# EntityOfCode/eoc-tfhe

Hardware: AMD Instinct MI355X
Metric: gate bootstraps/sec (HomNAND) (higher is better)
Workload: dtype f64

## Files before the change

eoc_tfhe_amd/csrc/kernels.hip.h:

```cpp
#pragma once
#include <hip/hip_runtime.h>
#include <stdint.h>
#include <type_traits>

namespace eoc {

typedef double d2 __attribute__((ext_vector_type(2)));

constexpr int kN = 1024;
constexpr int kNH = 512;
constexpr int kScr = 568;
constexpr int kTwF1 = 0;
constexpr int kTwF2 = 32;
constexpr int kTwI1 = 32 + 256;
constexpr int kTwI0 = 32 + 256 + 32;
constexpr int kTwEntries = 32 + 256 + 32 + 256;

#define EOC_FMA(a, b, c) __builtin_fma((a), (b), (c))

#define EOC_SQRT_HALF 0x1.6a09e667f3bcdp-1
#define EOC_E128_RE 0x1.d906bcf328d46p-1
#define EOC_E128_IM 0x1.87de2a6aea963p-2
#define EOC_E64_RE 0x1.f6297cff75cb0p-1
#define EOC_E64_IM 0x1.8f8b83c69a60bp-3
// ... 759 lines not shown
        EOC_SGB(EOC_M_DSW, 1);
        EOC_SGB(EOC_M_VALU, 5);
    }
    EOC_SGB(EOC_M_VALU, 16);
    EOC_SGB(EOC_M_DSR, 8);
    EOC_SB();
#pragma unroll
    for (int r = 0; r < 8; r++) scr[f12(lane * 8 + r)] = xb[r];
    wave_lds_fence();
    t21_read(xb, scr, lane);
    tw_load(t0, tw + kTwI0 + lane, 64);
    wave_lds_fence();
    inv_pass10(xa, t1);
#pragma unroll
    for (int k = 0; k < 8; k++) {
        EOC_SGB(EOC_M_DSW, 1);
        EOC_SGB(EOC_M_VALU, 4);
    }
    EOC_SGB(EOC_M_DSR, 12);
    EOC_SGB(EOC_M_VALU, 40);
    EOC_SB();
#pragma unroll
    for (int r = 0; r < 8; r++) scr[72 * hi + 8 * r + lo] = xa[r];
    wave_lds_fence();
    t10_read(xa, scr, lane);
    inv_pass10(xb, t1);
#pragma unroll
    for (int k = 0; k < 8; k++) {
        EOC_SGB(EOC_M_DSW, 1);
        EOC_SGB(EOC_M_VALU, 4);
    }
    EOC_SGB(EOC_M_DSR, 8);
    EOC_SGB(EOC_M_VALU, 40);
    EOC_SB();
#pragma unroll
    for (int r = 0; r < 8; r++) scr[72 * hi + 8 * r + lo] = xb[r];
    wave_lds_fence();
    t10_read(xb, scr, lane);
#pragma unroll
    for (int r = 0; r < 8; r++) ut[r] = s_twist[lane + 64 * r];
    wave_lds_fence();
    inv_pass10(xa, t0);
#pragma unroll
    for (int k = 0; k < 8; k++) {
        EOC_SGB(EOC_M_DSW, 1);
        EOC_SGB(EOC_M_VALU, 4);
    }
    EOC_SGB(EOC_M_DSR, 16);
    EOC_SGB(EOC_M_VALU, 40);
    EOC_SB();
    inv_pass10(xb, t0);
}

constexpr int kBRWideJobsPerWG = 2;
constexpr int kBRWideLds = (kTwEntries + kNH + kBRWideJobsPerWG * kScr) * 16 + kBRWideJobsPerWG * kAbarLds;


template <int BGBIT = 0, bool SABAR = false>
__global__ __launch_bounds__(64 * kBRWideJobsPerWG, 2) void k_blind_rotate_wide(BRArgs A, const d2 *__restrict__ g_tw,
                                                              const d2 *__restrict__ g_twist)
{
    constexpr bool TV = false, MANY = false, ENC = false;
    const int32_t *const tv = nullptr;
    const uint32_t tv_rows = 1, n_tables = 1;
#include "blind_rotate_wide.inc"
}
template <int BGBIT = 0, bool SABAR = false>
__global__ __launch_bounds__(64 * kBRWideJobsPerWG, 2) void k_blind_rotate_wide_tv(BRArgs A, const d2 *__restrict__ g_tw,
                                                                 const d2 *__restrict__ g_twist,
                                                                 const int32_t *__restrict__ tv, uint32_t tv_rows)
{
    constexpr bool TV = true, MANY = false, ENC = false;
    const uint32_t n_tables = 1;
#include "blind_rotate_wide.inc"
}
template <int BGBIT = 0, bool SABAR = false>
__global__ __launch_bounds__(64 * kBRWideJobsPerWG, 2) void k_lut_many_wide(BRArgs A, const d2 *__restrict__ g_tw,
                                                                            const d2 *__restrict__ g_twist,
                                                                            const int32_t *__restrict__ tv, uint32_t tv_rows,
                                                                            uint32_t n_tables)
{
    constexpr bool TV = true, MANY = true, ENC = false;
#include "blind_rotate_wide.inc"
}
template <int BGBIT = 0, bool SABAR = false>
__global__ __launch_bounds__(64 * kBRWideJobsPerWG, 2) void k_br_enc_wide(BRArgs A, const d2 *__restrict__ g_tw,
                                                                          const d2 *__restrict__ g_twist,
                                                                          const int32_t *__restrict__ tv, uint32_t tv_rows)
{
    constexpr bool TV = true, MANY = false, ENC = true;
    const uint32_t n_tables = 1;
#include "blind_rotate_wide.inc"
}

constexpr int KS_GT = 64;

struct KSArgs {
    const int32_t *ksk;
    const int32_t *u;
    uint32_t *ubar;
    int n, n1p, t, basebit;
    uint32_t S;
    GateDesc desc0;
    int inline_desc;
    int32_t mu;
};

__global__ __launch_bounds__(256) void k_ks_init(const GateDesc *__restrict__ descs, KSArgs A)
{
    const GateDesc d = A.inline_desc ? A.desc0 : descs[blockIdx.y];
    const uint32_t s = blockIdx.x;
    const uint32_t job = d.job_base + s;
    const int32_t *u1 = A.u + (size_t)job * (kN + 1);
    const bool mux = d.op == OP_MUX;
    const int32_t *u2 = u1 + (size_t)A.S * (kN + 1);
    const uint32_t prec_offset = 1u << (32 - (1 + A.basebit * A.t));
    for (int j = threadIdx.x; j < kN; j += 256) {
        uint32_t v = (uint32_t)u1[j];
        if (mux) v += (uint32_t)u2[j];
        A.ubar[(size_t)job * kN + j] = v + prec_offset;
    }
    int32_t *o = d.out + (size_t)s * (A.n + 1);
    for (int m = threadIdx.x; m < A.n; m += 256) o[m] = 0;
    if (threadIdx.x == 0) {
        uint32_t b = (uint32_t)u1[kN];
        if (mux) b += (uint32_t)u2[kN] + (uint32_t)A.mu;
        o[A.n] = (int32_t)b;
    }
}

typedef int i4 __attribute__((ext_vector_type(4)));

template <int T, int NWV, int IW>
struct KS3Cfg {
    static constexpr int NT = 64 * NWV;
    static constexpr int ROWI = 64 + 4;
    static constexpr int TABI = 16 * ROWI;
    static constexpr int WAVE_I = 2 * TABI;
    static constexpr int RED_I = 64 * ROWI;
    static constexpr int TAB_BYTES = NWV * WAVE_I * 4, RED_BYTES = (NWV > 1 ? NWV / 2 : 1) * RED_I * 4;
    static constexpr int LDS_BYTES = TAB_BYTES > RED_BYTES ? TAB_BYTES : RED_BYTES;
    static constexpr int NPAIR = T / 2;
    static constexpr int NSTAGE = IW * NPAIR;
    static constexpr int SLICE_I = NWV * IW;
    static constexpr int NS = kN / SLICE_I;
};

template <int T, int NWV, int IW>
__global__ __launch_bounds__(64 * NWV, 4) void k_keyswitch_waves(const GateDesc *__restrict__ descs, KSArgs A)
{
    typedef KS3Cfg<T, NWV, IW> C;
    static_assert(T % 2 == 0 && kN % C::SLICE_I == 0 && (NWV & (NWV - 1)) == 0, "shape");
    static_assert((NWV * C::WAVE_I - C::TABI) * 4 < 65536, "ds_write_addtid_b32 takes its base from M0[15:0]");
    extern __shared__ __attribute__((aligned(16))) unsigned char smem[];
    int *s_all = reinterpret_cast<int *>(smem);
    if ((uint32_t)(uintptr_t)smem != 0u) __builtin_trap();

    const GateDesc d = A.inline_desc ? A.desc0 : descs[blockIdx.y];
    const uint32_t ntiles = (A.S + 63) / 64, ncb = (uint32_t)A.n1p / 64u;
    const uint32_t tile = blockIdx.x % ntiles, rest = blockIdx.x / ntiles;
    const uint32_t cb = rest % ncb, slice = rest / ncb;
    const uint32_t s0 = tile * 64;
    const int tid = threadIdx.x, lane = tid & 63;
    const int w = __builtin_amdgcn_readfirstlane(tid >> 6);
    const bool valid = s0 + lane < A.S;
    const uint32_t job = d.job_base + (valid ? s0 + lane : A.S - 1);
    const int i0 = (int)slice * C::SLICE_I + w * IW;

    int *s_tab = s_all + w * C::WAVE_I;
    const size_t n1p = (size_t)A.n1p;
    int kr[6];
    for (int k = lane; k < 2 * C::ROWI; k += 64) s_tab[(k / C::ROWI) * C::TABI + k % C::ROWI] = 0;
    const uint32_t tab_lds = (uint32_t)(uintptr_t)s_tab;
    auto stage_load = [&](int st) {
        const int i = i0 + st / C::NPAIR, j0 = 2 * (st % C::NPAIR);
        const int *src = A.ksk + ((size_t)i * T + j0) * 3 * n1p + cb * 64 + lane;
#pragma unroll
        for (int k = 0; k < 6; k++) kr[k] = src[k * n1p];
    };
#define EOC_KS_ROW(BUF, D1, D2) ((BUF) * C::TABI * 4 + ((D1) * 4 + (D2)) * C::ROWI * 4)
    auto stage_store = [&](int buf) {
        const int a1 = kr[0], a2 = kr[1], a3 = kr[2], b1 = kr[3], b2 = kr[4], b3 = kr[5];
        const uint32_t base = tab_lds + (uint32_t)buf * (C::TABI * 4);
        uint32_t m0_saved;
        asm volatile("s_mov_b32 %0, m0\n\t"
                     "s_mov_b32 m0, %1\n\t"
                     "s_nop 1\n\t"
                     "ds_write_addtid_b32 %2 offset:%17\n\t"
                     "ds_write_addtid_b32 %3 offset:%18\n\t"
                     "ds_write_addtid_b32 %4 offset:%19\n\t"
                     "ds_write_addtid_b32 %5 offset:%20\n\t"
                     "ds_write_addtid_b32 %6 offset:%21\n\t"
                     "ds_write_addtid_b32 %7 offset:%22\n\t"
                     "ds_write_addtid_b32 %8 offset:%23\n\t"
                     "ds_write_addtid_b32 %9 offset:%24\n\t"
                     "ds_write_addtid_b32 %10 offset:%25\n\t"
                     "ds_write_addtid_b32 %11 offset:%26\n\t"
                     "ds_write_addtid_b32 %12 offset:%27\n\t"
                     "ds_write_addtid_b32 %13 offset:%28\n\t"
                     "ds_write_addtid_b32 %14 offset:%29\n\t"
                     "ds_write_addtid_b32 %15 offset:%30\n\t"
                     "ds_write_addtid_b32 %16 offset:%31\n\t"
                     "s_mov_b32 m0, %0"
                     : "=&s"(m0_saved)
                     : "s"(base), "v"(b1), "v"(b2), "v"(b3), "v"(a1), "v"(a1 + b1), "v"(a1 + b2), "v"(a1 + b3), "v"(a2),
                       "v"(a2 + b1), "v"(a2 + b2), "v"(a2 + b3), "v"(a3), "v"(a3 + b1), "v"(a3 + b2), "v"(a3 + b3),
                       "n"(EOC_KS_ROW(0, 0, 1)), "n"(EOC_KS_ROW(0, 0, 2)), "n"(EOC_KS_ROW(0, 0, 3)), "n"(EOC_KS_ROW(0, 1, 0)),
                       "n"(EOC_KS_ROW(0, 1, 1)), "n"(EOC_KS_ROW(0, 1, 2)), "n"(EOC_KS_ROW(0, 1, 3)), "n"(EOC_KS_ROW(0, 2, 0)),
                       "n"(EOC_KS_ROW(0, 2, 1)), "n"(EOC_KS_ROW(0, 2, 2)), "n"(EOC_KS_ROW(0, 2, 3)), "n"(EOC_KS_ROW(0, 3, 0)),
                       "n"(EOC_KS_ROW(0, 3, 1)), "n"(EOC_KS_ROW(0, 3, 2)), "n"(EOC_KS_ROW(0, 3, 3))
                     : "memory");
    };
#undef EOC_KS_ROW

    i4 acc[16];
#pragma unroll
    for (int c = 0; c < 16; c++) acc[c] = (i4){0, 0, 0, 0};

    stage_load(0);
    stage_store(0);
    wave_lds_fence();
    typedef uint32_t u4 __attribute__((ext_vector_type(4)));
    const u4 *ubp = reinterpret_cast<const u4 *>(A.ubar + (size_t)job * kN + i0);
    u4 ub4 = ubp[0];
#pragma unroll 1
    for (int ii = 0; ii < IW; ii++) {
        const int k4 = ii & 3;
        const uint32_t ub = k4 == 0 ? ub4.x : (k4 == 1 ? ub4.y : (k4 == 2 ? ub4.z : ub4.w));
        u4 ub4n = ub4;
        if (k4 == 3 && ii + 1 < IW) ub4n = ubp[(ii + 1) >> 2];
#pragma unroll 1
        for (int q = 0; q < C::NPAIR; q++) {
            const int st = ii * C::NPAIR + q;
            const int buf = st & 1;
            stage_load(st + 1 < C::NSTAGE ? st + 1 : st);
            const uint32_t nib = (ub >> (28 - 4 * q)) & 15u;
            const i4 *row = reinterpret_cast<const i4 *>(s_tab + buf * C::TABI + (int)nib * C::ROWI);
#pragma unroll
            for (int c0 = 0; c0 < 16; c0 += 8) {
                i4 v[8];
#pragma unroll
                for (int c = 0; c < 8; c++) v[c] = row[c0 + c];
#pragma unroll
                for (int c = 0; c < 8; c++) acc[c0 + c] -= v[c];
                __builtin_amdgcn_sched_barrier(0);
            }
            stage_store(buf ^ 1);
            wave_lds_fence();
        }
        ub4 = ub4n;
    }

    __syncthreads();
#pragma unroll
    for (int h = NWV / 2; h >= 1; h /= 2) {
        if (w >= h && w < 2 * h) {
            int *r = s_all + (w - h) * C::RED_I + lane * C::ROWI;
#pragma unroll
            for (int c = 0; c < 16; c++) *reinterpret_cast<i4 *>(r + 4 * c) = acc[c];
        }
        __syncthreads();
        if (w < h) {
            const int *r = s_all + w * C::RED_I + lane * C::ROWI;
#pragma unroll
            for (int c = 0; c < 16; c++) acc[c] += *reinterpret_cast<const i4 *>(r + 4 * c);
        }
        __syncthreads();
    }
    if (w == 0) {
        int *r = s_all + lane * C::ROWI;
#pragma unroll
        for (int c = 0; c < 16; c++) *reinterpret_cast<i4 *>(r + 4 * c) = acc[c];
    }
    __syncthreads();
    const int col = (int)cb * 64 + lane;
#pragma unroll 4
    for (int k = 0; k < 64 / NWV; k++) {
        const int ct = w * (64 / NWV) + k;
        const int v = s_all[ct * C::ROWI + lane];
        if (v != 0 && s0 + ct < A.S && col <= A.n) atomicAdd(d.out + (size_t)(s0 + ct) * (A.n + 1) + col, v);
    }
}

__global__ __launch_bounds__(256) void k_keyswitch_generic(const GateDesc *__restrict__ descs, KSArgs A)
{
    const GateDesc d = A.inline_desc ? A.desc0 : descs[blockIdx.y];
    const uint32_t s = blockIdx.x, job = d.job_base + s;
    const int base1 = (1 << A.basebit) - 1;
    int32_t *o = d.out + (size_t)s * (A.n + 1);
    for (int m = threadIdx.x; m <= A.n; m += 256) {
        uint32_t acc = (uint32_t)o[m];
        for (int i = 0; i < kN; i++) {
            const uint32_t ub = A.ubar[(size_t)job * kN + i];
            for (int j = 0; j < A.t; j++) {
                const uint32_t dg = (ub >> (32 - (j + 1) * A.basebit)) & (uint32_t)base1;
                if (dg) acc -= (uint32_t)A.ksk[(((size_t)i * A.t + j) * base1 + (dg - 1)) * A.n1p + m];
            }
        }
        o[m] = (int32_t)acc;
    }
}

typedef int i16 __attribute__((ext_vector_type(16)));
constexpr int KSM_KI = 4;

template <int NWV>
__global__ __launch_bounds__(64 * NWV, 2) void k_keyswitch_mfma(const GateDesc *__restrict__ descs, KSArgs A,
                                                                 const i4 *__restrict__ limbs, int nsl)
{
    constexpr int MT = 64 * NWV;
    constexpr int CHUNKS = KSM_KI * 4;
    constexpr int NLD = CHUNKS / NWV;
    static_assert(CHUNKS % NWV == 0, "shape");
    __shared__ i4 s_b[2][CHUNKS * 64];

    const GateDesc d = A.inline_desc ? A.desc0 : descs[blockIdx.y];
    const uint32_t ntiles = (A.S + MT - 1) / MT, nct = (uint32_t)A.n1p / 32u;
    const uint32_t tile = blockIdx.x % ntiles, rest = blockIdx.x / ntiles;
    const uint32_t ct = rest % nct, slice = rest / nct;
    const int per = kN / nsl, nstage = per / KSM_KI;
    const int ibeg = (int)slice * per;
    const int tid = threadIdx.x, lane = tid & 63, r = lane & 31, h = lane >> 5;
    const int w = __builtin_amdgcn_readfirstlane(tid >> 6);
    const uint32_t row0 = tile * MT + (uint32_t)w * 64u;

    typedef uint32_t u4 __attribute__((ext_vector_type(4)));
    const u4 *ubp[2];
#pragma unroll
    for (int m = 0; m < 2; m++) {
        const uint32_t s = row0 + 32u * m + r;
        const uint32_t job = d.job_base + (s < A.S ? s : A.S - 1);
        ubp[m] = reinterpret_cast<const u4 *>(A.ubar + (size_t)job * kN + ibeg);
    }
    const i4 *bsrc = limbs + ((size_t)ibeg * nct + ct) * 256 + lane;
    i4 stg[NLD];
    auto stage_load = [&](int st) {
#pragma unroll
        for (int x = 0; x < NLD; x++) {
            const int c = w + NWV * x;
            stg[x] = bsrc[((size_t)(st * KSM_KI + (c >> 2)) * nct) * 256 + (c & 3) * 64];
        }
    };
    auto stage_store = [&](int buf) {
#pragma unroll
        for (int x = 0; x < NLD; x++) s_b[buf][(w + NWV * x) * 64 + lane] = stg[x];
    };

    i16 acc[2][4];
#pragma unroll
    for (int m = 0; m < 2; m++)
#pragma unroll
        for (int k = 0; k < 4; k++)
#pragma unroll
            for (int q = 0; q < 16; q++) acc[m][k][q] = 0;

    stage_load(0);
    u4 ubc[2] = {ubp[0][0], ubp[1][0]};
    stage_store(0);
    stage_load(nstage > 1 ? 1 : 0);
    __syncthreads();
    const int sh0 = 27 - 8 * h;
#pragma unroll 1
    for (int st = 0; st < nstage; st++) {
        const int buf = st & 1;
        const int stn = st + 1 < nstage ? st + 1 : st;
        const u4 ubn[2] = {ubp[0][stn], ubp[1][stn]};
#pragma unroll
        for (int ki = 0; ki < KSM_KI; ki++) {
            i4 b[4], a[2];
#pragma unroll
            for (int k = 0; k < 4; k++) b[k] = s_b[buf][(ki * 4 + k) * 64 + lane];
#pragma unroll
            for (int m = 0; m < 2; m++) {
                const uint32_t ub = ubc[m][ki];
#pragma unroll
                for (int q = 0; q < 4; q++) a[m][q] = (int)(1u << ((ub >> (sh0 - 2 * q)) & 24u));
            }
#pragma unroll
            for (int m = 0; m < 2; m++)
#pragma unroll
                for (int k = 0; k < 4; k++)
                    acc[m][k] = __builtin_amdgcn_mfma_i32_32x32x32_i8(a[m], b[k], acc[m][k], 0, 0, 0);
        }
        stage_store(buf ^ 1);
        stage_load(st + 2 < nstage ? st + 2 : nstage - 1);
        __syncthreads();
        ubc[0] = ubn[0];
        ubc[1] = ubn[1];
    }

    const int col = (int)ct * 32 + r;
    if (col <= A.n) {
#pragma unroll
        for (int m = 0; m < 2; m++)
#pragma unroll
            for (int q = 0; q < 16; q++) {
                const uint32_t s = row0 + 32u * m + (uint32_t)((q & 3) + 8 * (q >> 2) + 4 * h);
                const uint32_t v = (uint32_t)acc[m][0][q] + ((uint32_t)acc[m][1][q] << 8) + ((uint32_t)acc[m][2][q] << 16) +
                                   ((uint32_t)acc[m][3][q] << 24);
                if (v != 0 && s < A.S) atomicAdd(d.out + (size_t)s * (A.n + 1) + col, (int)(0u - v));
            }
    }
}

__global__ __launch_bounds__(256) void k_ksk_limbs(const int32_t *__restrict__ ksk, uint32_t *__restrict__ limbs, int n1p)
{
    const uint32_t nct = (uint32_t)n1p / 32u;
    const uint32_t limb = blockIdx.x & 3u, ct = (blockIdx.x >> 2) % nct, i = (blockIdx.x >> 2) / nct;
    const int q = threadIdx.x & 3, lane = threadIdx.x >> 2, r = lane & 31, h = lane >> 5;
    const int j = 4 * h + q;
    const int32_t *row = ksk + ((size_t)i * 8 + j) * 3 * n1p + ct * 32 + r;
    uint32_t o = 0;
#pragma unroll
    for (int dg = 1; dg <= 3; dg++) {
        int32_t v = row[(size_t)(dg - 1) * n1p];
        int32_t l = 0;
        for (uint32_t k = 0; k <= limb; k++) {
            l = (int32_t)(((uint32_t)v + 128u) & 255u) - 128;
            v = (int32_t)((uint32_t)v - (uint32_t)l) >> 8;
        }
        o |= ((uint32_t)l & 255u) << (8 * dg);
    }
    limbs[(size_t)blockIdx.x * 256 + threadIdx.x] = o;
}

static inline size_t ks_limb_bytes(int n1p) { return (size_t)kN * (size_t)(n1p / 32) * 4096; }
static inline void ks_limbs_launch(const int32_t *ksk, void *limbs, int n1p, hipStream_t st)
{
    hipLaunchKernelGGL(k_ksk_limbs, dim3((unsigned)(kN * (n1p / 32) * 4)), dim3(256), 0, st, ksk,
                       static_cast<uint32_t *>(limbs), n1p);
}

struct KSMPlan {
    int nwv, nsl;
    unsigned gx;
};
static inline KSMPlan ks_mfma_plan(uint32_t S, int n1p)
{
    KSMPlan p;
    p.nwv = 4;
    const unsigned ntiles = (S + 64 * p.nwv - 1) / (64 * p.nwv), nct = (unsigned)n1p / 32u;
    p.nsl = 1;
    while (p.nsl < 32 && ntiles * nct * p.nsl * p.nwv < 2048u) p.nsl *= 2;
    p.gx = ntiles * nct * (unsigned)p.nsl;
    return p;
}
static inline void ks_mfma_launch(const KSMPlan &pl, uint32_t ngates, const GateDesc *descs, const KSArgs &a,
                                  const void *limbs, hipStream_t st)
{
    const i4 *lp = static_cast<const i4 *>(limbs);
    if (pl.nwv == 8)
        hipLaunchKernelGGL(k_keyswitch_mfma<8>, dim3(pl.gx, ngates), dim3(512), 0, st, descs, a, lp, pl.nsl);
    else
        hipLaunchKernelGGL(k_keyswitch_mfma<4>, dim3(pl.gx, ngates), dim3(256), 0, st, descs, a, lp, pl.nsl);
}

constexpr int kCompactSlotsPerWG = 16;
__global__ __launch_bounds__(256) void k_compact_expand(const int32_t *__restrict__ lists, uint64_t first, uint32_t S,
                                                        uint32_t *__restrict__ ubar, int32_t *__restrict__ out, int n,
                                                        uint32_t prec_offset)
{
    static_assert(kN % kCompactSlotsPerWG == 0, "a workgroup's slots lie inside one list");
    __shared__ int32_t s_c0[kN];
    const uint64_t g0 = (first / kCompactSlotsPerWG + blockIdx.x) * kCompactSlotsPerWG;
    const int32_t *list = lists + (g0 / kN) * (uint64_t)(2 * kN);
    for (int k = threadIdx.x; k < kN; k += 256) s_c0[k] = list[k];
    __syncthreads();
    for (int q = 0; q < kCompactSlotsPerWG; q++) {
        const uint64_t g = g0 + q;
        if (g < first || g >= first + S) continue;
        const uint32_t s = (uint32_t)(g - first);
        const int j = (int)(g % kN);
        uint32_t *row = ubar + (size_t)s * kN;
        for (int i = threadIdx.x; i < kN; i += 256) {
            const uint32_t v = (uint32_t)s_c0[(j - i) & (kN - 1)];
            row[i] = (i <= j ? v : 0u - v) + prec_offset;
        }
        int32_t *o = out + (size_t)s * (n + 1);
        for (int m = threadIdx.x; m < n; m += 256) o[m] = 0;
        if (threadIdx.x == 0) o[n] = list[kN + j];
    }
}

constexpr int kCmuxItemsPerWG = 2;
constexpr int kCmuxLds = (kTwEntries + kNH + 2 * kCmuxItemsPerWG * kScr) * 16;

struct CmuxArgs {
    const d2 *sel;
    const int32_t *in0, *in1;
    int32_t *out;
    size_t sel_x, sel_y;
    size_t in0_x, in0_y, in1_x, in1_y, out_x, out_y;
    uint32_t nx;
    int rot;
    int Bgbit;
};

template <int L> __device__ __forceinline__ void load_selector_row(const d2 *sel, int h, int lane, int p, int c, d2 (&b)[8])
{
    const d2 *row = sel + ((size_t)(h * L + (p - 1)) * 2 + c) * kNH + lane;
#pragma unroll
    for (int r = 0; r < 8; r++) b[r] = row[r * 64];
}
__device__ __forceinline__ uint2 leveled_words(const d2 &s, const d2 &u)
{
    const d2 y = cmulc(s, u);
    return make_uint2(wrap_trunc(y.x), wrap_trunc(y.y));
}
#define EOC_NEGACYCLIC(idx, v) (((idx) & kN) ? 0u - (v) : (v))

template <int L, int BGBIT = 0>
__global__ __launch_bounds__(128 * kCmuxItemsPerWG, 2) void k_cmux(CmuxArgs A, const d2 *__restrict__ g_tw,
                                                                    const d2 *__restrict__ g_twist)
{
#define EOC_LEVELED_PART 1
#include "leveled_pair.inc"
    const int32_t *pa = A.in0 + ix * A.in0_x + iy * A.in0_y + (size_t)h * kN;
    const int32_t *pb = A.in1 + ix * A.in1_x + iy * A.in1_y + (size_t)h * kN;
    const d2 *sel = A.sel + ix * A.sel_x + iy * A.sel_y;
#define EOC_LEVELED_PART 2
#include "leveled_pair.inc"
#pragma unroll
    for (int r = 0; r < 16; r++) {
        const int j = lane + 64 * (r & 7) + (r >> 3) * kNH;
        const int idx = (j - A.rot) & (2 * kN - 1);
        const uint32_t b = (uint32_t)pb[idx & (kN - 1)];
        const uint32_t v = offset + EOC_NEGACYCLIC(idx, b) - (uint32_t)pa[j];
        if (r < 8) dlo[r] = v;
        else dhi[r - 8] = v;
    }
#define EOC_LEVELED_PART 3
#include "leveled_pair.inc"
    int32_t *po = A.out + ix * A.out_x + iy * A.out_y + (size_t)h * kN;
#pragma unroll
    for (int r = 0; r < 8; r++) {
        const int j = lane + 64 * r;
        const uint2 e = leveled_words(S[r], ut[r]);
        po[j] = (int32_t)((uint32_t)pa[j] + e.x);
        po[j + kNH] = (int32_t)((uint32_t)pa[j + kNH] + e.y);
    }
}

__global__ __launch_bounds__(256) void k_tlwe_extract(const int32_t *__restrict__ lists, size_t list_stride, uint32_t W,
                                                      uint32_t *__restrict__ ubar, int32_t *__restrict__ out, int n,
                                                      uint32_t prec_offset)
{
    __shared__ int32_t s_c0[kN];
    const int32_t *list = lists + (size_t)blockIdx.y * list_stride;
    for (int k = threadIdx.x; k < kN; k += 256) s_c0[k] = list[k];
    __syncthreads();
    for (int q = 0; q < kCompactSlotsPerWG; q++) {
        const uint32_t j = blockIdx.x * kCompactSlotsPerWG + q;
        if (j >= W) break;
        const size_t s = (size_t)blockIdx.y * W + j;
        uint32_t *row = ubar + s * kN;
        for (int i = threadIdx.x; i < kN; i += 256) {
            const uint32_t v = (uint32_t)s_c0[((int)j - i) & (kN - 1)];
            row[i] = (i <= (int)j ? v : 0u - v) + prec_offset;
        }
        int32_t *o = out + s * (n + 1);
        for (int m = threadIdx.x; m < n; m += 256) o[m] = 0;
        if (threadIdx.x == 0) o[n] = list[kN + j];
    }
}

constexpr int kPackT = 4, kPackBasebit = 4;
constexpr int kPackChunk = 16;
constexpr int kPackTile = 64;

__global__ __launch_bounds__(256) void k_pack_gather(const int32_t *__restrict__ in, size_t count, int n,
                                                     int32_t *__restrict__ cols, int32_t *__restrict__ lists)
{
    __shared__ int32_t s_tile[kPackTile][kPackTile + 1];
    const int tx = threadIdx.x & 63, ty = threadIdx.x >> 6;
    const int i0 = blockIdx.x * kPackTile, m0 = blockIdx.y * kPackTile;
    const size_t list = blockIdx.z, s0 = list * kN + i0;
    for (int r = ty; r < kPackTile; r += 4) {
        const size_t s = s0 + r;
        const int m = m0 + tx;
        s_tile[r][tx] = (s < count && m <= n) ? in[s * ((size_t)n + 1) + m] : 0;
    }
    __syncthreads();
    for (int r = ty; r < kPackTile; r += 4) {
        const int m = m0 + r;
        const int32_t v = s_tile[tx][r];
        if (m < n) cols[(list * n + m) * kN + i0 + tx] = v;
        else if (m == n) lists[list * 2 * kN + kN + i0 + tx] = v;
    }
    if (blockIdx.y == 0 && ty == 0) lists[list * 2 * kN + i0 + tx] = 0;
}

constexpr int kPackWavesPerWG = 4;
constexpr int kPackLds = (kTwEntries + kNH + kPackWavesPerWG * kScr) * 16;

__global__ __launch_bounds__(64 * kPackWavesPerWG, 2) void k_pack_rows(const int32_t *__restrict__ cols,
                                                                       const d2 *__restrict__ key, int32_t *__restrict__ lists,
                                                                       int n, uint32_t nchunks, uint32_t items,
                                                                       const d2 *__restrict__ g_tw,
                                                                       const d2 *__restrict__ g_twist)
{
    extern __shared__ __attribute__((aligned(16))) unsigned char smem[];
    d2 *s_tw = reinterpret_cast<d2 *>(smem);
    d2 *s_twist = s_tw + kTwEntries;
    const int tid = threadIdx.x, lane = tid & 63;
    const int wv = __builtin_amdgcn_readfirstlane(tid >> 6);
    d2 *scr = s_twist + kNH + wv * kScr;
    load_tables(s_tw, s_twist, g_tw, g_twist, tid, 64 * kPackWavesPerWG);
    __syncthreads();
    const uint32_t item = blockIdx.x * kPackWavesPerWG + (uint32_t)wv;
    if (item >= items) return;
    const uint32_t list = item / nchunks, chunk = item - list * nchunks;
    const int m_first = (int)chunk * kPackChunk, m_end = min(m_first + kPackChunk, n);

    const Gadget<kPackBasebit> gd = make_gadget<kPackBasebit>(0);
    uint32_t offset = 1u << (31 - kPackT * kPackBasebit);
#pragma unroll
    for (int p = 1; p <= kPackT; p++) offset += gd.halfBg << gd.shift(p);

    uint32_t dlo[8], dhi[8];
    auto make_x0 = [&](int p, d2 (&x)[8]) __attribute__((always_inline)) { digit_pass(dlo, dhi, gd.shift(p), gd, x); };
    d2 S0[8], S1[8];
    auto key_index = [&](int m, auto first_tag) __attribute__((always_inline)) {
        constexpr bool kFirst = decltype(first_tag)::value;
        const int32_t *pa = cols + ((size_t)list * n + m) * kN;
#pragma unroll
        for (int r = 0; r < 8; r++) {
            dlo[r] = (uint32_t)pa[lane + 64 * r] + offset;
            dhi[r] = (uint32_t)pa[lane + 64 * r + kNH] + offset;
        }
        const d2 *rows = key + (size_t)m * kPackT * 2 * kNH + lane;
        d2 xa[8], xb[8];
#pragma unroll
        for (int j0 = 1; j0 < kPackT; j0 += 2) {
            make_x0(j0, xa);
            fft_fwd_rest_x2(xa, xb, [&]() __attribute__((always_inline)) { make_x0(j0 + 1, xb); }, s_tw, scr, lane);
#pragma unroll
            for (int r = 0; r < 8; r++) {
                const d2 a0 = rows[((j0 - 1) * 2 + 0) * kNH + r * 64], a1 = rows[((j0 - 1) * 2 + 1) * kNH + r * 64];
                const d2 b0 = rows[(j0 * 2 + 0) * kNH + r * 64], b1 = rows[(j0 * 2 + 1) * kNH + r * 64];
                const d2 s0 = (kFirst && j0 == 1) ? cmul0(xa[r], a0) : cmac1(xa[r], a0, S0[r]);
                const d2 s1 = (kFirst && j0 == 1) ? cmul0(xa[r], a1) : cmac1(xa[r], a1, S1[r]);
                S0[r] = cmac1(xb[r], b0, s0);
                S1[r] = cmac1(xb[r], b1, s1);
            }
        }
    };
    key_index(m_first, std::true_type());
#pragma unroll 1
    for (int m = m_first + 1; m < m_end; m++) key_index(m, std::false_type());

    int32_t *po = lists + (size_t)list * 2 * kN;
    d2 ut[8];
    fft_inv_wave(S0, ut, s_tw, s_twist, scr, lane);
#pragma unroll
    for (int r = 0; r < 8; r++) {
        const int j = lane + 64 * r;
        const d2 y = cmulc(S0[r], ut[r]);
        atomicAdd(po + j, (int)(0u - wrap_trunc(y.x)));
        atomicAdd(po + j + kNH, (int)(0u - wrap_trunc(y.y)));
    }
    fft_inv_wave(S1, ut, s_tw, s_twist, scr, lane);
#pragma unroll
    for (int r = 0; r < 8; r++) {
        const int j = lane + 64 * r;
        const d2 y = cmulc(S1[r], ut[r]);
        atomicAdd(po + kN + j, (int)(0u - wrap_trunc(y.x)));
        atomicAdd(po + kN + j + kNH, (int)(0u - wrap_trunc(y.y)));
    }
}

template <int p>
__global__ __launch_bounds__(256) void k_tvpack_cols(const int32_t *__restrict__ in, uint32_t rows, uint32_t list0, int n,
                                                     int32_t *__restrict__ cols, int32_t *__restrict__ lists)
{
    static_assert(p == 2 || p == 4 || p == 8, "window boundaries are multiples of the tile only for these");
    const int tx = threadIdx.x & 63, ty = threadIdx.x >> 6;
    const int i0 = blockIdx.x * kPackTile, m0 = blockIdx.y * kPackTile;
    const size_t list = blockIdx.z;
    const uint32_t gl = list0 + (uint32_t)list, f = gl / rows, s = gl - f * rows;
    const bool neg = i0 >= kN - kN / (2 * p);
    const int j = neg ? 0 : (i0 * p + kN / 2) / kN;
    const int32_t *row = in + (((size_t)f * p + j) * rows + s) * ((size_t)n + 1);
    const int m = m0 + tx;
    const uint32_t w = m <= n ? (uint32_t)row[m] : 0u;
    const int32_t mine = (int32_t)(neg ? 0u - w : w);
    for (int r = ty; r < kPackTile; r += 4) {
        const int mr = m0 + r;
        const int32_t v = __shfl(mine, r, 64);
        if (mr < n) cols[(list * n + mr) * kN + i0 + tx] = v;
        else if (mr == n) lists[list * 2 * kN + kN + i0 + tx] = v;
    }
    if (blockIdx.y == 0 && ty == 0) lists[list * 2 * kN + i0 + tx] = 0;
}

struct DemuxArgs {
    const d2 *sel;
    const int32_t *in;
    int32_t *out0, *out1;
    size_t sel_x, sel_y;
    size_t in_x, in_y, out_x, out_y;
    uint32_t nx;
    int accumulate;
    int Bgbit;
};

template <int L, int BGBIT = 0>
__global__ __launch_bounds__(128 * kCmuxItemsPerWG, 2) void k_demux(DemuxArgs A, const d2 *__restrict__ g_tw,
                                                                     const d2 *__restrict__ g_twist)
{
#define EOC_LEVELED_PART 1
#include "leveled_pair.inc"
    const int32_t *px = A.in + ix * A.in_x + iy * A.in_y + (size_t)h * kN;
    const d2 *sel = A.sel + ix * A.sel_x + iy * A.sel_y;
#define EOC_LEVELED_PART 2
#include "leveled_pair.inc"
#pragma unroll
    for (int r = 0; r < 8; r++) {
        dlo[r] = offset + (uint32_t)px[lane + 64 * r];
        dhi[r] = offset + (uint32_t)px[lane + 64 * r + kNH];
    }
#define EOC_LEVELED_PART 3
#include "leveled_pair.inc"
    const size_t oo = ix * A.out_x + iy * A.out_y + (size_t)h * kN;
    int32_t *p0 = A.out0 + oo, *p1 = A.out1 + oo;
    if (A.accumulate) {
#pragma unroll
        for (int r = 0; r < 8; r++) {
            const int j = lane + 64 * r;
            const uint2 e = leveled_words(S[r], ut[r]);
            atomicAdd(p1 + j, (int)e.x);
            atomicAdd(p1 + j + kNH, (int)e.y);
            atomicAdd(p0 + j, (int)((uint32_t)px[j] - e.x));
            atomicAdd(p0 + j + kNH, (int)((uint32_t)px[j + kNH] - e.y));
        }
    } else {
#pragma unroll
        for (int r = 0; r < 8; r++) {
            const int j = lane + 64 * r;
            const uint2 e = leveled_words(S[r], ut[r]);
            p1[j] = (int32_t)e.x;
            p1[j + kNH] = (int32_t)e.y;
            p0[j] = (int32_t)((uint32_t)px[j] - e.x);
            p0[j + kNH] = (int32_t)((uint32_t)px[j + kNH] - e.y);
        }
    }
}
// ... 281 lines not shown
```

Baseline: 332,500.

## Repack keyswitch key limbs to cut MFMA count in keyswitch kernel

Changes the keyswitch MFMA formulation so that each 32-wide K slice spans the 3 nonzero digit values of 4 key indices times 4 digit positions. It does this by packing limbs per quad of i and per digit value, instead of using a one-hot shift encoding with zero-padding per digit. The A operand is now a 0/1 byte mask built from the 2-bit digits, so one K=32 MFMA covers more useful work, and fewer limb bytes are loaded. KSM_KI doubles and the slice-count heuristic is retuned. The limb precompute kernel changes to match the new layout, which raises the risk of indexing errors.

After: 332,300. Within noise of the previous version (-0.1%).

```diff
diff --git a/eoc_tfhe_amd/csrc/kernels.hip.h b/eoc_tfhe_amd/csrc/kernels.hip.h
--- a/eoc_tfhe_amd/csrc/kernels.hip.h
+++ b/eoc_tfhe_amd/csrc/kernels.hip.h
@@ -1085,16 +1085,18 @@
 }
 
 typedef int i16 __attribute__((ext_vector_type(16)));
-constexpr int KSM_KI = 4;
+constexpr int KSM_KI = 8;
+constexpr int KSM_QF = 12;
 
 template <int NWV>
 __global__ __launch_bounds__(64 * NWV, 2) void k_keyswitch_mfma(const GateDesc *__restrict__ descs, KSArgs A,
                                                                  const i4 *__restrict__ limbs, int nsl)
 {
     constexpr int MT = 64 * NWV;
-    constexpr int CHUNKS = KSM_KI * 4;
+    constexpr int NQ = KSM_KI / 4;
+    constexpr int CHUNKS = NQ * KSM_QF;
     constexpr int NLD = CHUNKS / NWV;
-    static_assert(CHUNKS % NWV == 0, "shape");
+    static_assert(CHUNKS % NWV == 0 && KSM_KI % 4 == 0, "shape");
     __shared__ i4 s_b[2][CHUNKS * 64];
 
     const GateDesc d = A.inline_desc ? A.desc0 : descs[blockIdx.y];
@@ -1115,13 +1117,13 @@
         const uint32_t job = d.job_base + (s < A.S ? s : A.S - 1);
         ubp[m] = reinterpret_cast<const u4 *>(A.ubar + (size_t)job * kN + ibeg);
     }
-    const i4 *bsrc = limbs + ((size_t)ibeg * nct + ct) * 256 + lane;
+    const i4 *bsrc = limbs + ((size_t)(ibeg / 4) * nct + ct) * (KSM_QF * 64) + lane;
     i4 stg[NLD];
     auto stage_load = [&](int st) {
 #pragma unroll
         for (int x = 0; x < NLD; x++) {
             const int c = w + NWV * x;
-            stg[x] = bsrc[((size_t)(st * KSM_KI + (c >> 2)) * nct) * 256 + (c & 3) * 64];
+            stg[x] = bsrc[((size_t)(st * NQ + c / KSM_QF) * nct) * (KSM_QF * 64) + (c % KSM_QF) * 64];
         }
     };
     auto stage_store = [&](int buf) {
@@ -1138,38 +1140,60 @@
             for (int q = 0; q < 16; q++) acc[m][k][q] = 0;
 
     stage_load(0);
-    u4 ubc[2] = {ubp[0][0], ubp[1][0]};
+    u4 ubc[2][NQ];
+#pragma unroll
+    for (int m = 0; m < 2; m++)
+#pragma unroll
+        for (int qd = 0; qd < NQ; qd++) ubc[m][qd] = ubp[m][qd];
     stage_store(0);
     stage_load(nstage > 1 ? 1 : 0);
     __syncthreads();
-    const int sh0 = 27 - 8 * h;
+    const uint32_t sh0 = 24u - 8u * (uint32_t)h;
 #pragma unroll 1
     for (int st = 0; st < nstage; st++) {
         const int buf = st & 1;
         const int stn = st + 1 < nstage ? st + 1 : st;
-        const u4 ubn[2] = {ubp[0][stn], ubp[1][stn]};
-#pragma unroll
-        for (int ki = 0; ki < KSM_KI; ki++) {
-            i4 b[4], a[2];
-#pragma unroll
-            for (int k = 0; k < 4; k++) b[k] = s_b[buf][(ki * 4 + k) * 64 + lane];
-#pragma unroll
-            for (int m = 0; m < 2; m++) {
-                const uint32_t ub = ubc[m][ki];
-#pragma unroll
-                for (int q = 0; q < 4; q++) a[m][q] = (int)(1u << ((ub >> (sh0 - 2 * q)) & 24u));
+        u4 ubn[2][NQ];
+#pragma unroll
+        for (int m = 0; m < 2; m++)
+#pragma unroll
+            for (int qd = 0; qd < NQ; qd++) ubn[m][qd] = ubp[m][stn * NQ + qd];
+#pragma unroll
+        for (int qd = 0; qd < NQ; qd++) {
+            int a[2][12];
+#pragma unroll
+            for (int m = 0; m < 2; m++)
+#pragma unroll
+                for (int ki = 0; ki < 4; ki++) {
+                    const uint32_t x = (ubc[m][qd][ki] >> sh0) & 255u;
+                    const uint32_t t = x | (x << 12);
+                    const uint32_t y = t | (t << 6);
+                    const uint32_t lo = y & 0x01010101u, hi = (y >> 1) & 0x01010101u, d3 = lo & hi;
+                    a[m][3 * ki + 0] = (int)(lo ^ d3);
+                    a[m][3 * ki + 1] = (int)(hi ^ d3);
+                    a[m][3 * ki + 2] = (int)d3;
+                }
+#pragma unroll
+            for (int k = 0; k < 4; k++) {
+                i4 b[3];
+#pragma unroll
+                for (int f = 0; f < 3; f++) b[f] = s_b[buf][((qd * 4 + k) * 3 + f) * 64 + lane];
+#pragma unroll
+                for (int m = 0; m < 2; m++)
+#pragma unroll
+                    for (int f = 0; f < 3; f++) {
+                        const i4 af = {a[m][4 * f], a[m][4 * f + 1], a[m][4 * f + 2], a[m][4 * f + 3]};
+                        acc[m][k] = __builtin_amdgcn_mfma_i32_32x32x32_i8(af, b[f], acc[m][k], 0, 0, 0);
+                    }
             }
-#pragma unroll
-            for (int m = 0; m < 2; m++)
-#pragma unroll
-                for (int k = 0; k < 4; k++)
-                    acc[m][k] = __builtin_amdgcn_mfma_i32_32x32x32_i8(a[m], b[k], acc[m][k], 0, 0, 0);
         }
         stage_store(buf ^ 1);
         stage_load(st + 2 < nstage ? st + 2 : nstage - 1);
         __syncthreads();
-        ubc[0] = ubn[0];
-        ubc[1] = ubn[1];
+#pragma unroll
+        for (int m = 0; m < 2; m++)
+#pragma unroll
+            for (int qd = 0; qd < NQ; qd++) ubc[m][qd] = ubn[m][qd];
     }
 
     const int col = (int)ct * 32 + r;
@@ -1189,28 +1213,29 @@
 __global__ __launch_bounds__(256) void k_ksk_limbs(const int32_t *__restrict__ ksk, uint32_t *__restrict__ limbs, int n1p)
 {
     const uint32_t nct = (uint32_t)n1p / 32u;
-    const uint32_t limb = blockIdx.x & 3u, ct = (blockIdx.x >> 2) % nct, i = (blockIdx.x >> 2) / nct;
-    const int q = threadIdx.x & 3, lane = threadIdx.x >> 2, r = lane & 31, h = lane >> 5;
-    const int j = 4 * h + q;
-    const int32_t *row = ksk + ((size_t)i * 8 + j) * 3 * n1p + ct * 32 + r;
+    const uint32_t fl = blockIdx.x % (uint32_t)KSM_QF, f = fl % 3u, limb = fl / 3u;
+    const uint32_t ct = (blockIdx.x / (uint32_t)KSM_QF) % nct, quad = (blockIdx.x / (uint32_t)KSM_QF) / nct;
+    const int e = threadIdx.x & 3, lane = threadIdx.x >> 2, r = lane & 31, h = lane >> 5;
+    const int g = 4 * (int)f + e, i = 4 * (int)quad + g / 3, dg = g % 3 + 1;
     uint32_t o = 0;
 #pragma unroll
-    for (int dg = 1; dg <= 3; dg++) {
-        int32_t v = row[(size_t)(dg - 1) * n1p];
+    for (int p = 0; p < 4; p++) {
+        const int j = 4 * h + 3 - p;
+        int32_t v = ksk[(((size_t)i * 8 + j) * 3 + (dg - 1)) * n1p + ct * 32 + r];
         int32_t l = 0;
         for (uint32_t k = 0; k <= limb; k++) {
             l = (int32_t)(((uint32_t)v + 128u) & 255u) - 128;
             v = (int32_t)((uint32_t)v - (uint32_t)l) >> 8;
         }
-        o |= ((uint32_t)l & 255u) << (8 * dg);
+        o |= ((uint32_t)l & 255u) << (8 * p);
     }
     limbs[(size_t)blockIdx.x * 256 + threadIdx.x] = o;
 }
 
-static inline size_t ks_limb_bytes(int n1p) { return (size_t)kN * (size_t)(n1p / 32) * 4096; }
+static inline size_t ks_limb_bytes(int n1p) { return (size_t)(kN / 4) * (size_t)(n1p / 32) * (KSM_QF * 1024); }
 static inline void ks_limbs_launch(const int32_t *ksk, void *limbs, int n1p, hipStream_t st)
 {
-    hipLaunchKernelGGL(k_ksk_limbs, dim3((unsigned)(kN * (n1p / 32) * 4)), dim3(256), 0, st, ksk,
+    hipLaunchKernelGGL(k_ksk_limbs, dim3((unsigned)((kN / 4) * (n1p / 32) * KSM_QF)), dim3(256), 0, st, ksk,
                        static_cast<uint32_t *>(limbs), n1p);
 }
 
@@ -1224,7 +1249,8 @@
     p.nwv = 4;
     const unsigned ntiles = (S + 64 * p.nwv - 1) / (64 * p.nwv), nct = (unsigned)n1p / 32u;
     p.nsl = 1;
-    while (p.nsl < 32 && ntiles * nct * p.nsl * p.nwv < 2048u) p.nsl *= 2;
+    while (p.nsl < 8 && ntiles * nct * p.nsl * p.nwv < 2048u) p.nsl *= 2;
+    while (p.nsl < 32 && ntiles * nct * p.nsl * p.nwv < 1024u) p.nsl *= 2;
     p.gx = ntiles * nct * (unsigned)p.nsl;
     return p;
 }
```
